# xmindflow/cenet

Hardware: AMD Instinct MI355X
Metric: training images/sec (224x224, 4-class) (higher is better)
Workload: dtype bf16

## Files before the change

cenet_amd/csrc/attn_diff.hip:

```cpp
#include "common.h"
#include "../../include/cenet_hip.h"
#include <cstdlib>

typedef bf16_t bf;
#define DA_NEG (-1.0e30f)
#define DA_LOG2E 1.4426950408889634f

#ifdef CENET_HOSTSIM_BUILD
__device__ __forceinline__ float da_exp2(float x) { return exp2f(x); }
__device__ __forceinline__ bool da_any(bool v) {
  int x = v ? 1 : 0;
#pragma unroll
  for (int o = 32; o > 0; o >>= 1) x |= __shfl_xor(x, o);
  return x != 0;
}
#else
__device__ __forceinline__ float da_exp2(float x) { return __builtin_amdgcn_exp2f(x); }
__device__ __forceinline__ bool da_any(bool v) { return __any(v); }
typedef short da_s4 __attribute__((ext_vector_type(4)));
#endif
__device__ __forceinline__ float da_max3(float a, float b, float c3) { return fmaxf(fmaxf(a, b), c3); }
__device__ __forceinline__ void da_wave_sync() {
#ifdef CENET_HOSTSIM_BUILD
  hipsim::wave_barrier();
#else
  __builtin_amdgcn_wave_barrier();
#endif
}

struct DiffArgs {
  const bf *q, *k, *v;
  bf* U;
  float* lse;
  const bf* dU;
  bf *dq, *dk, *dv;
  bf* aug;
  int B, H, N, hd;
  float scale;
  int bmul;
};

struct DaChunk {
  const bf* g;
  int lrow;
  int loff;
  unsigned fill;
};
__device__ __forceinline__ void da_fetch(const DaChunk& c, long tile_step, int rows_left, unsigned (&r)[4]) {
  r[0] = c.fill;
  r[1] = r[2] = r[3] = 0u;
  if (c.g && c.lrow < rows_left) memcpy(r, c.g + tile_step, 16);
  else if (!c.g) r[0] = 0u;
}
__device__ __forceinline__ bf16x8 da_rm(const bf* img, int pitch, int row, int col, int hh) {
  bf16x8 f;
  memcpy(&f, img + row * pitch + col + 8 * hh, 16);
  return f;
}
__device__ __forceinline__ bf16x8 da_tr(const bf* img, int pitch, int s2, int C0, int lane) {
  const int hh = lane >> 5;
  bf16x8 f;
#ifdef CENET_HOSTSIM_BUILD
  const int r = lane & 31;
#pragma unroll
  for (int j = 0; j < 8; ++j) f[j] = (short)img[(16 * s2 + 8 * (j >> 2) + 4 * hh + (j & 3)) * pitch + C0 + r];
#else
  const int g2 = (lane >> 4) & 1, i = lane & 15, q = i >> 2, p = i & 3;
  const bf* a0 = img + (16 * s2 + 4 * hh + q) * pitch + C0 + 16 * g2 + 4 * p;
  const da_s4 lo = __builtin_amdgcn_ds_read_tr16_b64_v4i16((da_s4 __attribute__((address_space(3)))*)a0);
  const da_s4 hi = __builtin_amdgcn_ds_read_tr16_b64_v4i16((da_s4 __attribute__((address_space(3)))*)(a0 + 8 * pitch));
  f[0] = lo[0], f[1] = lo[1], f[2] = lo[2], f[3] = lo[3];
  f[4] = hi[0], f[5] = hi[1], f[6] = hi[2], f[7] = hi[3];
#endif
  return f;
}
__device__ __forceinline__ bf16x8 da_ld8(const bf* p, bool ok) {
  bf16x8 f = {0, 0, 0, 0, 0, 0, 0, 0};
  if (ok) memcpy(&f, p, 16);
  return f;
}
__device__ __forceinline__ void da_half(unsigned (&r)[4], int s) {
  if (s) r[0] = r[2], r[1] = r[3];
  r[2] = r[3] = 0u;
}
__device__ __forceinline__ bf16x8 da_ld4h(const bf* pair, int s, bool ok) {
  unsigned u[4] = {0u, 0u, 0u, 0u};
  if (ok) {
    memcpy(u, pair, 16);
    da_half(u, s);
  }
  bf16x8 f;
  memcpy(&f, u, 16);
  return f;
}
__device__ __forceinline__ bf16x8 da_pack8(const f32x16& x, int s) {
  unsigned u[4];
#pragma unroll
  for (int j = 0; j < 4; ++j) u[j] = cenet_pack_bf2(x[8 * s + 2 * j], x[8 * s + 2 * j + 1]);
  bf16x8 f;
  memcpy(&f, u, 16);
  return f;
}
__device__ __forceinline__ int da_row(int reg, int hh) { return (reg & 3) + 8 * (reg >> 2) + 4 * hh; }
__device__ __forceinline__ f32x16 da_zero() {
  f32x16 z;
#pragma unroll
  for (int i = 0; i < 16; ++i) z[i] = 0.f;
  return z;
}
struct da_true { static constexpr bool value = true; };
struct da_false { static constexpr bool value = false; };
#define DA_MFMA(a, b, c) __builtin_amdgcn_mfma_f32_32x32x16_bf16((a), (b), (c), 0, 0, 0)

__device__ __forceinline__ void da_split3(float x, unsigned short* o) {
  const unsigned h = cenet_f2bf(x);
  const float r1 = x - cenet_bf2f(h);
  const unsigned m = cenet_f2bf(r1);
  const unsigned l = cenet_f2bf(r1 - cenet_bf2f(m));
  o[0] = (unsigned short)h, o[1] = (unsigned short)m, o[2] = (unsigned short)l;
}

template <int HDP>
struct DaGeo {
  static constexpr int DVP = 2 * HDP;
  static constexpr int KP = 2 * HDP + 8;
  static constexpr int VPT = DVP;
  static constexpr int VPR = DVP + 8;
  static constexpr int CK = 2 * HDP / 8, CV = DVP / 8;
};

template <int HDP, int QT, int MINB, bool ONE, bool H4 = false>
__global__ __launch_bounds__(256, MINB) void dattn_fwd_kernel(DiffArgs a) {
  typedef DaGeo<HDP> G;
  constexpr int NKS = HDP / 16, NDT = G::DVP / 32, NH = ONE ? 1 : 2;
  constexpr int KIMG = 32 * G::KP, VIMG = 32 * G::VPT + 64, IMG = KIMG + VIMG;
  constexpr int NCH = 32 * (G::CK + G::CV), CPT = (NCH + 255) / 256;
  __shared__ __attribute__((aligned(16))) bf lds[2 * IMG];
  const int tid = threadIdx.x, lane = tid & 63, wave = tid >> 6, r = lane & 31, hh = lane >> 5;
  const cenet_bid bid = cenet_xcd_block();
  const int b = bid.y / a.H, h = bid.y - b * a.H;
  const int q0 = (bid.x * 4 + wave) * (32 * QT);
  const int N = a.N, hd = a.hd, dv = 2 * hd, E = 2 * a.H * hd;
  const float c = a.scale * DA_LOG2E;
  const bf* qb = a.q + (long)b * a.bmul * N * E;
  const bf* kb = a.k + (long)b * a.bmul * N * E;
  const bf* vb = a.v + (long)b * a.bmul * N * (a.H * dv) + h * dv;

  DaChunk ch[CPT];
  int hs[CPT];
#pragma unroll
  for (int j = 0; j < CPT; ++j) {
    const int id = tid + 256 * j;
    ch[j].fill = 0u;
    hs[j] = -1;
    if (id >= NCH) {
      ch[j].g = nullptr;
      ch[j].lrow = 0;
      ch[j].loff = -1;
    } else if (id < 32 * G::CK) {
      const int row = id / G::CK, cc = id - row * G::CK, s = cc / (HDP / 8), c8 = cc - s * (HDP / 8);
      ch[j].lrow = row;
      ch[j].loff = row * G::KP + s * HDP + 8 * c8;
      ch[j].g = H4 ? (c8 == 0 ? kb + (long)row * E + 2 * h * hd : nullptr)
                   : (8 * c8 < hd ? kb + (long)row * E + (2 * h + s) * hd + 8 * c8 : nullptr);
      hs[j] = s;
    } else {
      const int id2 = id - 32 * G::CK, row = id2 / G::CV, c8 = id2 - row * G::CV;
      ch[j].lrow = row;
      ch[j].loff = KIMG + row * G::VPT + 8 * c8;
      ch[j].g = 8 * c8 < dv ? vb + (long)row * (a.H * dv) + 8 * c8 : nullptr;
    }
  }
  unsigned pre[CPT][4];
  auto fetch = [&](int k0) __attribute__((always_inline)) {
#pragma unroll
    for (int j = 0; j < CPT; ++j) {
      da_fetch(ch[j], (long)k0 * (ch[j].loff < KIMG ? E : a.H * dv), N - k0, pre[j]);
      if (H4 && hs[j] >= 0) da_half(pre[j], hs[j]);
    }
  };
  auto stage = [&](int buf) __attribute__((always_inline)) {
#pragma unroll
    for (int j = 0; j < CPT; ++j)
      if (ch[j].loff >= 0) memcpy(lds + buf * IMG + ch[j].loff, pre[j], 16);
  };

  bf16x8 qf[QT][2][NKS];
  f32x16 O[QT][NH][NDT];
  float m[QT][NH], l[QT][NH];
#pragma unroll
  for (int t = 0; t < QT; ++t) {
    const int qi = q0 + 32 * t + r < N ? q0 + 32 * t + r : N - 1;
#pragma unroll
    for (int s = 0; s < 2; ++s) {
#pragma unroll
      for (int ks = 0; ks < NKS; ++ks)
        qf[t][s][ks] = H4 ? da_ld4h(qb + (long)qi * E + 2 * h * hd, s, hh == 0)
                          : da_ld8(qb + (long)qi * E + (2 * h + s) * hd + 16 * ks + 8 * hh, 16 * ks + 8 * hh < hd);
    }
#pragma unroll
    for (int s = 0; s < NH; ++s) {
#pragma unroll
      for (int dt = 0; dt < NDT; ++dt) O[t][s][dt] = da_zero();
      m[t][s] = DA_NEG;
      l[t][s] = 0.f;
    }
  }
  fetch(0);
  stage(0);
  __syncthreads();
  int cur = 0;
  for (int k0 = 0; k0 < N; k0 += 32) {
    const bool more = k0 + 32 < N;
    if (more) fetch(k0 + 32);
    const bf* Kimg = lds + cur * IMG;
    const bf* Vimg = Kimg + KIMG;
    const int klim = N - k0;
    auto tile = [&](auto masked) __attribute__((always_inline)) {
      constexpr bool MASKED = decltype(masked)::value;
      constexpr bool LATE = HDP > 32;
      bf16x8 kf[LATE ? 1 : 2][NKS], vf[LATE ? 1 : NDT][2];
      if (!LATE) {
#pragma unroll
        for (int s = 0; s < 2; ++s)
#pragma unroll
          for (int ks = 0; ks < NKS; ++ks) kf[LATE ? 0 : s][ks] = da_rm(Kimg, G::KP, r, s * HDP + 16 * ks, hh);
#pragma unroll
        for (int dt = 0; dt < NDT; ++dt)
#pragma unroll
          for (int s2 = 0; s2 < 2; ++s2) vf[LATE ? 0 : dt][s2] = da_tr(Vimg, G::VPT, s2, 32 * dt, lane);
      }
#pragma unroll
      for (int t = 0; t < QT; ++t)
#pragma unroll
        for (int s = 0; s < NH; ++s) {
          f32x16 S = da_zero();
#pragma unroll
          for (int sp = (ONE ? 0 : s); sp <= (ONE ? 1 : s); ++sp)
#pragma unroll
            for (int ks = 0; ks < NKS; ++ks)
              S = DA_MFMA(LATE ? da_rm(Kimg, G::KP, r, sp * HDP + 16 * ks, hh) : kf[LATE ? 0 : sp][ks], qf[t][sp][ks], S);
          if (MASKED) {
#pragma unroll
            for (int i = 0; i < 16; ++i)
              if (da_row(i, hh) >= klim) S[i] = DA_NEG;
          }
          float mx = da_max3(S[0], S[1], S[2]);
#pragma unroll
          for (int i = 3; i < 15; i += 2) mx = da_max3(mx, S[i], S[i + 1]);
          mx = fmaxf(mx, S[15]);
          mx = fmaxf(mx, __shfl_xor(mx, 32));
          if (da_any(mx > m[t][s])) {
            const float mn = fmaxf(m[t][s], mx);
            const float alpha = da_exp2((m[t][s] - mn) * c);
            m[t][s] = mn;
            l[t][s] *= alpha;
#pragma unroll
            for (int dt = 0; dt < NDT; ++dt)
#pragma unroll
              for (int i = 0; i < 16; ++i) O[t][s][dt][i] *= alpha;
          }
          const float mc = m[t][s] * c;
          float rs = 0.f;
#pragma unroll
          for (int i = 0; i < 16; ++i) {
            const float p = da_exp2(S[i] * c - mc);
            S[i] = p;
            rs += p;
          }
          l[t][s] += rs;
          const bf16x8 p0 = da_pack8(S, 0), p1 = da_pack8(S, 1);
#pragma unroll
          for (int dt = 0; dt < NDT; ++dt) {
            O[t][s][dt] = DA_MFMA(LATE ? da_tr(Vimg, G::VPT, 0, 32 * dt, lane) : vf[LATE ? 0 : dt][0], p0, O[t][s][dt]);
            O[t][s][dt] = DA_MFMA(LATE ? da_tr(Vimg, G::VPT, 1, 32 * dt, lane) : vf[LATE ? 0 : dt][1], p1, O[t][s][dt]);
          }
        }
    };
    if (q0 < N) {
      if (klim < 32) tile(da_true());
      else tile(da_false());
    }
    if (more) stage(cur ^ 1);
    __syncthreads();
    cur ^= 1;
  }
  if (q0 >= N) return;
#pragma unroll
  for (int t = 0; t < QT; ++t) {
    const int qi = q0 + 32 * t + r;
#pragma unroll
    for (int s = 0; s < NH; ++s) {
      const float lt = l[t][s] + __shfl_xor(l[t][s], 32);
      const long hrow = ((long)b * NH * a.H + NH * h + s) * N + qi;
      if (qi < N) {
        const float inv = 1.f / lt;
        bf* up = a.U + hrow * dv;
#pragma unroll
        for (int dt = 0; dt < NDT; ++dt)
#pragma unroll
          for (int g = 0; g < 4; ++g) {
            const int f0 = 32 * dt + 8 * g + 4 * hh;
            if (f0 < dv) {
              float o[4];
#pragma unroll
              for (int i = 0; i < 4; ++i) o[i] = O[t][s][dt][4 * g + i] * inv;
              st4v(up + f0, o);
            }
          }
        if (hh == 0) a.lse[hrow] = m[t][s] * a.scale + logf(lt);
      }
    }
  }
}

template <int HDP, bool ONE, bool H4 = false>
__global__ __launch_bounds__(256, HDP > 32 ? 1 : (HDP <= 16 ? 3 : 2)) void dattn_bwd_dq_kernel(DiffArgs a) {
  typedef DaGeo<HDP> G;
  constexpr int NKS = HDP / 16, NKD = G::DVP / 16, NH = ONE ? 1 : 2;
  constexpr int NFT = (HDP + 31) / 32;
  constexpr int KIMG = 32 * G::KP + 64, VIMG = 32 * G::VPR, IMG = KIMG + VIMG;
  constexpr int NCH = 32 * (G::CK + G::CV), CPT = (NCH + 255) / 256;
  __shared__ __attribute__((aligned(16))) bf lds[2 * IMG];
  const int tid = threadIdx.x, lane = tid & 63, wave = tid >> 6, r = lane & 31, hh = lane >> 5;
  const cenet_bid bid = cenet_xcd_block();
  const int b = bid.y / a.H, h = bid.y - b * a.H;
  const int q0 = (bid.x * 4 + wave) * 32;
  const int N = a.N, hd = a.hd, dv = 2 * hd, E = 2 * a.H * hd;
  const float c = a.scale * DA_LOG2E;
  const bf* qb = a.q + (long)b * a.bmul * N * E;
  const bf* kb = a.k + (long)b * a.bmul * N * E;
  const bf* vb = a.v + (long)b * a.bmul * N * (a.H * dv) + h * dv;
  const int qi = q0 + r < N ? q0 + r : N - 1;

  DaChunk ch[CPT];
  int hs[CPT];
#pragma unroll
  for (int j = 0; j < CPT; ++j) {
    const int id = tid + 256 * j;
    ch[j].fill = 0u;
    hs[j] = -1;
    if (id >= NCH) {
      ch[j].g = nullptr;
      ch[j].lrow = 0;
      ch[j].loff = -1;
    } else if (id < 32 * G::CK) {
      const int row = id / G::CK, cc = id - row * G::CK, s = cc / (HDP / 8), c8 = cc - s * (HDP / 8);
      ch[j].lrow = row;
      ch[j].loff = row * G::KP + s * HDP + 8 * c8;
      ch[j].g = H4 ? (c8 == 0 ? kb + (long)row * E + 2 * h * hd : nullptr)
                   : (8 * c8 < hd ? kb + (long)row * E + (2 * h + s) * hd + 8 * c8 : nullptr);
      hs[j] = s;
    } else {
      const int id2 = id - 32 * G::CK, row = id2 / G::CV, c8 = id2 - row * G::CV;
      ch[j].lrow = row;
      ch[j].loff = KIMG + row * G::VPR + 8 * c8;
      ch[j].g = 8 * c8 < dv ? vb + (long)row * (a.H * dv) + 8 * c8 : nullptr;
    }
  }
  unsigned pre[CPT][4];
  auto fetch = [&](int k0) __attribute__((always_inline)) {
#pragma unroll
    for (int j = 0; j < CPT; ++j) {
      da_fetch(ch[j], (long)k0 * (ch[j].loff < KIMG ? E : a.H * dv), N - k0, pre[j]);
      if (H4 && hs[j] >= 0) da_half(pre[j], hs[j]);
    }
  };
  auto stage = [&](int buf) __attribute__((always_inline)) {
#pragma unroll
    for (int j = 0; j < CPT; ++j)
      if (ch[j].loff >= 0) memcpy(lds + buf * IMG + ch[j].loff, pre[j], 16);
  };

  bf16x8 qf[2][NKS], gf[NH][NKD];
  float lse2[NH], dl[NH];
  f32x16 dq[2][NFT];
#pragma unroll
  for (int s = 0; s < 2; ++s) {
#pragma unroll
    for (int ks = 0; ks < NKS; ++ks)
      qf[s][ks] = H4 ? da_ld4h(qb + (long)qi * E + 2 * h * hd, s, hh == 0)
                     : da_ld8(qb + (long)qi * E + (2 * h + s) * hd + 16 * ks + 8 * hh, 16 * ks + 8 * hh < hd);
#pragma unroll
    for (int ft = 0; ft < NFT; ++ft) dq[s][ft] = da_zero();
  }
#pragma unroll
  for (int s = 0; s < NH; ++s) {
    const long hrow = ((long)b * NH * a.H + NH * h + s) * N + qi;
    float acc = 0.f;
#pragma unroll
    for (int kd = 0; kd < NKD; ++kd) {
      const bool ok = 16 * kd + 8 * hh < dv;
      gf[s][kd] = da_ld8(a.dU + hrow * dv + 16 * kd + 8 * hh, ok);
      const bf16x8 uf = da_ld8(a.U + hrow * dv + 16 * kd + 8 * hh, ok);
#pragma unroll
      for (int j = 0; j < 8; ++j) acc += cenet_bf2f((unsigned short)gf[s][kd][j]) * cenet_bf2f((unsigned short)uf[j]);
    }
    acc += __shfl_xor(acc, 32);
    dl[s] = acc;
    const float lse = a.lse[hrow];
    lse2[s] = lse * DA_LOG2E;
    if (q0 + r < N) {
      unsigned short row8[8] = {0, 0, 0, 0, 0, 0, 0, 0};
      da_split3(hh == 0 ? lse / a.scale : acc, row8);
      memcpy(a.aug + hrow * 16 + 8 * hh, row8, 16);
    }
  }
  fetch(0);
  stage(0);
  __syncthreads();
  int cur = 0;
  for (int k0 = 0; k0 < N; k0 += 32) {
    const bool more = k0 + 32 < N;
    if (more) fetch(k0 + 32);
    const bf* Kimg = lds + cur * IMG;
    const bf* Vimg = Kimg + KIMG;
    const int klim = N - k0;
    auto tile = [&](auto masked) __attribute__((always_inline)) {
      constexpr bool MASKED = decltype(masked)::value;
      bf16x8 vf[NKD];
#pragma unroll
      for (int kd = 0; kd < NKD; ++kd) vf[kd] = da_rm(Vimg, G::VPR, r, 16 * kd, hh);
#pragma unroll
      for (int s = 0; s < NH; ++s) {
        constexpr bool INITD = HDP > 16;
        f32x16 S = da_zero(), dP;
#pragma unroll
        for (int i = 0; i < 16; ++i) dP[i] = INITD ? -dl[s] : 0.f;
#pragma unroll
        for (int sp = (ONE ? 0 : s); sp <= (ONE ? 1 : s); ++sp)
#pragma unroll
          for (int ks = 0; ks < NKS; ++ks) S = DA_MFMA(da_rm(Kimg, G::KP, r, sp * HDP + 16 * ks, hh), qf[sp][ks], S);
#pragma unroll
        for (int kd = 0; kd < NKD; ++kd) dP = DA_MFMA(vf[kd], gf[s][kd], dP);
#pragma unroll
        for (int i = 0; i < 16; ++i) {
          float p = da_exp2(S[i] * c - lse2[s]);
          if (MASKED && da_row(i, hh) >= klim) p = 0.f;
          S[i] = INITD ? p * dP[i] : p * (dP[i] - dl[s]);
        }
#pragma unroll
        for (int sp = (ONE ? 0 : s); sp <= (ONE ? 1 : s); ++sp)
#pragma unroll
          for (int s2 = 0; s2 < 2; ++s2) {
            const bf16x8 dsB = da_pack8(S, s2);
#pragma unroll
            for (int ft = 0; ft < NFT; ++ft)
              dq[sp][ft] = DA_MFMA(da_tr(Kimg, G::KP, s2, sp * HDP + 32 * ft, lane), dsB, dq[sp][ft]);
          }
      }
    };
    if (q0 < N) {
      if (klim < 32) tile(da_true());
      else tile(da_false());
    }
    if (more) stage(cur ^ 1);
    __syncthreads();
    cur ^= 1;
  }
  if (q0 + r < N) {
#pragma unroll
    for (int s = 0; s < 2; ++s) {
      bf* dp = a.dq + ((long)b * a.bmul * N + qi) * E + (2 * h + s) * hd;
#pragma unroll
      for (int ft = 0; ft < NFT; ++ft)
#pragma unroll
        for (int g = 0; g < (HDP < 32 ? HDP / 8 : 4); ++g) {
          const int d0 = 32 * ft + 8 * g + 4 * hh;
          if (d0 < hd) {
            float o[4];
#pragma unroll
            for (int i = 0; i < 4; ++i) o[i] = dq[s][ft][4 * g + i] * a.scale;
            st4v(dp + d0, o);
          }
        }
    }
  }
}

template <int HDP, bool ONE, bool H4 = false>
__global__ __launch_bounds__(256, HDP > 32 ? 1 : 2) void dattn_bwd_dkv_kernel(DiffArgs a) {
  typedef DaGeo<HDP> G;
  constexpr int NKS = HDP / 16, NKD = G::DVP / 16, NDT = G::DVP / 32, NH = ONE ? 1 : 2;
  constexpr int NFT = (HDP + 31) / 32;
  constexpr int AP = 40;
  constexpr int QIMG = 32 * G::KP + 64, GIMG = 32 * G::VPR + 64, AIMG = 32 * AP, IMG = QIMG + NH * GIMG + AIMG;
  constexpr int NCH = 32 * (G::CK + NH * G::CV + 2 * NH), CPT = (NCH + 255) / 256;
  __shared__ __attribute__((aligned(16))) bf lds[2 * IMG];
  const int tid = threadIdx.x, lane = tid & 63, wave = tid >> 6, r = lane & 31, hh = lane >> 5;
  const cenet_bid bid = cenet_xcd_block();
  const int b = bid.y / a.H, h = bid.y - b * a.H;
  const int k0 = (bid.x * 4 + wave) * 32;
  const int N = a.N, hd = a.hd, dv = 2 * hd, E = 2 * a.H * hd;
  const float c = a.scale * DA_LOG2E;
  const bf* qb = a.q + (long)b * a.bmul * N * E;
  const bf* kb = a.k + (long)b * a.bmul * N * E;
  const bf* vb = a.v + (long)b * a.bmul * N * (a.H * dv) + h * dv;
  const long hb0 = ((long)b * NH * a.H + NH * h) * N;
  const int ki = k0 + r < N ? k0 + r : N - 1;

  DaChunk ch[CPT];
  long gstep[CPT];
  int hs[CPT];
#pragma unroll
  for (int j = 0; j < CPT; ++j) {
    int id = tid + 256 * j;
    ch[j].fill = 0u;
    hs[j] = -1;
    gstep[j] = 0;
    if (id >= NCH) {
      ch[j].g = nullptr;
      ch[j].lrow = 0;
      ch[j].loff = -1;
    } else if (id < 32 * G::CK) {
      const int row = id / G::CK, cc = id - row * G::CK, s = cc / (HDP / 8), c8 = cc - s * (HDP / 8);
      ch[j].lrow = row;
      ch[j].loff = row * G::KP + s * HDP + 8 * c8;
      ch[j].g = H4 ? (c8 == 0 ? qb + (long)row * E + 2 * h * hd : nullptr)
                   : (8 * c8 < hd ? qb + (long)row * E + (2 * h + s) * hd + 8 * c8 : nullptr);
      hs[j] = s;
      gstep[j] = 32L * E;
    } else if ((id -= 32 * G::CK) < NH * 32 * G::CV) {
      const int s = id / (32 * G::CV), id2 = id - s * 32 * G::CV, row = id2 / G::CV, c8 = id2 - row * G::CV;
      ch[j].lrow = row;
      ch[j].loff = QIMG + s * GIMG + row * G::VPR + 8 * c8;
      ch[j].g = 8 * c8 < dv ? a.dU + (hb0 + (long)s * N + row) * dv + 8 * c8 : nullptr;
      gstep[j] = 32L * dv;
    } else {
      id -= NH * 32 * G::CV;
      const int row = id / (2 * NH), s = (id - row * 2 * NH) >> 1, kind = id & 1;
      ch[j].lrow = row;
      ch[j].loff = QIMG + NH * GIMG + row * AP + s * 16 + 8 * kind;
      ch[j].g = a.aug + (hb0 + (long)s * N + row) * 16 + 8 * kind;
      ch[j].fill = kind == 0 ? 0x7149u : 0u;
      gstep[j] = 32L * 16;
    }
  }
  unsigned pre[CPT][4];
  auto fetch = [&](int q0) __attribute__((always_inline)) {
#pragma unroll
    for (int j = 0; j < CPT; ++j) {
      da_fetch(ch[j], (q0 >> 5) * gstep[j], N - q0, pre[j]);
      if (H4 && hs[j] >= 0) da_half(pre[j], hs[j]);
    }
  };
  auto stage = [&](int buf) __attribute__((always_inline)) {
#pragma unroll
    for (int j = 0; j < CPT; ++j)
      if (ch[j].loff >= 0) memcpy(lds + buf * IMG + ch[j].loff, pre[j], 16);
  };

  bf16x8 kfB[2][NKS], vfB[NKD];
#pragma unroll
  for (int s = 0; s < 2; ++s)
#pragma unroll
    for (int ks = 0; ks < NKS; ++ks)
      kfB[s][ks] = H4 ? da_ld4h(kb + (long)ki * E + 2 * h * hd, s, hh == 0)
                      : da_ld8(kb + (long)ki * E + (2 * h + s) * hd + 16 * ks + 8 * hh, 16 * ks + 8 * hh < hd);
#pragma unroll
  for (int kd = 0; kd < NKD; ++kd) vfB[kd] = da_ld8(vb + (long)ki * (a.H * dv) + 16 * kd + 8 * hh, 16 * kd + 8 * hh < dv);
  bf16x8 negB = {0, 0, 0, 0, 0, 0, 0, 0};
  if (hh == 0) negB[0] = negB[1] = negB[2] = (short)0xBF80;
  f32x16 dK[2][NFT], dV[NDT];
#pragma unroll
  for (int s = 0; s < 2; ++s)
#pragma unroll
    for (int ft = 0; ft < NFT; ++ft) dK[s][ft] = da_zero();
#pragma unroll
  for (int dt = 0; dt < NDT; ++dt) dV[dt] = da_zero();

  fetch(0);
  stage(0);
  __syncthreads();
  int cur = 0;
  for (int q0 = 0; q0 < N; q0 += 32) {
    const bool more = q0 + 32 < N;
    if (more) fetch(q0 + 32);
    const bf* Qimg = lds + cur * IMG;
    const bf* Aimg = Qimg + QIMG + NH * GIMG;
    if (k0 < N) {
#pragma unroll
      for (int s = 0; s < NH; ++s) {
        const bf* Gimg = Qimg + QIMG + s * GIMG;
        f32x16 S = da_zero(), dP = da_zero();
#pragma unroll
        for (int sp = (ONE ? 0 : s); sp <= (ONE ? 1 : s); ++sp)
#pragma unroll
          for (int ks = 0; ks < NKS; ++ks) S = DA_MFMA(da_rm(Qimg, G::KP, r, sp * HDP + 16 * ks, hh), kfB[sp][ks], S);
#pragma unroll
        for (int kd = 0; kd < NKD; ++kd) dP = DA_MFMA(da_rm(Gimg, G::VPR, r, 16 * kd, hh), vfB[kd], dP);
        bf16x8 al = {0, 0, 0, 0, 0, 0, 0, 0}, ad = {0, 0, 0, 0, 0, 0, 0, 0};
        if (hh == 0) {
          memcpy(&al, Aimg + r * AP + s * 16, 16);
          memcpy(&ad, Aimg + r * AP + s * 16 + 8, 16);
        }
        S = DA_MFMA(al, negB, S);
        dP = DA_MFMA(ad, negB, dP);
#pragma unroll
        for (int i = 0; i < 16; ++i) {
          const float p = da_exp2(S[i] * c);
          S[i] = p;
          dP[i] = p * dP[i];
        }
#pragma unroll
        for (int s2 = 0; s2 < 2; ++s2) {
          const bf16x8 pB = da_pack8(S, s2), dsB = da_pack8(dP, s2);
#pragma unroll
          for (int dt = 0; dt < NDT; ++dt) dV[dt] = DA_MFMA(da_tr(Gimg, G::VPR, s2, 32 * dt, lane), pB, dV[dt]);
#pragma unroll
          for (int sp = (ONE ? 0 : s); sp <= (ONE ? 1 : s); ++sp)
#pragma unroll
            for (int ft = 0; ft < NFT; ++ft)
              dK[sp][ft] = DA_MFMA(da_tr(Qimg, G::KP, s2, sp * HDP + 32 * ft, lane), dsB, dK[sp][ft]);
        }
      }
    }
    if (more) stage(cur ^ 1);
    __syncthreads();
    cur ^= 1;
  }
  if (k0 + r < N) {
#pragma unroll
    for (int s = 0; s < 2; ++s) {
      bf* dp = a.dk + ((long)b * a.bmul * N + ki) * E + (2 * h + s) * hd;
#pragma unroll
      for (int ft = 0; ft < NFT; ++ft)
#pragma unroll
        for (int g = 0; g < (HDP < 32 ? HDP / 8 : 4); ++g) {
          const int d0 = 32 * ft + 8 * g + 4 * hh;
          if (d0 < hd) {
            float o[4];
#pragma unroll
            for (int i = 0; i < 4; ++i) o[i] = dK[s][ft][4 * g + i] * a.scale;
            st4v(dp + d0, o);
          }
        }
    }
    bf* dvp = a.dv + ((long)b * a.bmul * N + ki) * (a.H * dv) + h * dv;
#pragma unroll
    for (int dt = 0; dt < NDT; ++dt)
#pragma unroll
      for (int g = 0; g < 4; ++g) {
        const int f0 = 32 * dt + 8 * g + 4 * hh;
        if (f0 < dv) {
          float o[4];
#pragma unroll
          for (int i = 0; i < 4; ++i) o[i] = dV[dt][4 * g + i];
          st4v(dvp + f0, o);
        }
      }
  }
}

extern "C" int cenet_diffattn_heads_supported(int hd, int N) {
  return (hd == 4 || hd == 8 || hd == 16 || hd == 32 || hd == 40 || hd == 64) && N >= 1;
}
static bool da_hd40_p64() {
  const char* e = getenv("CENET_DATTN_HD40_HDP64");
  return e && e[0] == '1';
}
extern "C" long cenet_diffattn_heads_ws_bytes(int B, int H, int N) { return (long)B * 2 * H * N * 16 * 2; }

static int da_fill(DiffArgs& a, const cenet_diffattn_t* p) {
  if (!p || !p->q || !p->k || !p->v || !p->U || !p->lse) return CENET_EINVAL;
  if (p->B <= 0 || p->H <= 0 || p->N <= 0 || !cenet_diffattn_heads_supported(p->hd, p->N)) return CENET_EUNSUPPORTED;
  a.q = (const bf*)p->q; a.k = (const bf*)p->k; a.v = (const bf*)p->v;
  a.U = (bf*)p->U; a.lse = p->lse; a.dU = (const bf*)p->dU;
  a.dq = (bf*)p->dq; a.dk = (bf*)p->dk; a.dv = (bf*)p->dv; a.aug = (bf*)p->ws;
  a.B = p->B; a.H = p->H; a.N = p->N; a.hd = p->hd; a.scale = p->scale;
  a.bmul = p->batch_mul > 0 ? p->batch_mul : 1;
  const uintptr_t m = (uintptr_t)a.q | (uintptr_t)a.k | (uintptr_t)a.v | (uintptr_t)a.U | (uintptr_t)a.dU | (uintptr_t)a.dq |
                      (uintptr_t)a.dk | (uintptr_t)a.dv | (uintptr_t)a.aug;
  if (m & 15) return CENET_EINVAL;
  return CENET_OK;
}

extern "C" int cenet_diffattn_heads_fwd_bf16(const cenet_diffattn_t* p, hipStream_t stream) {
  DiffArgs a;
  const int rc = da_fill(a, p);
  if (rc != CENET_OK) return rc;
  const int bh = a.B * a.H;
  if (a.hd == 4) {
    CENET_LAUNCH((dattn_fwd_kernel<16, 1, 3, false, true>), dim3(cdiv(a.N, 128), bh), dim3(256), stream, a);
  } else if (a.hd <= 16) {
    static const int v = getenv("CENET_DATTN_QT2") ? 2 : 1;
    if (v == 2 && a.N >= 1024) CENET_LAUNCH((dattn_fwd_kernel<16, 2, 2, false>), dim3(cdiv(a.N, 256), bh), dim3(256), stream, a);
    else CENET_LAUNCH((dattn_fwd_kernel<16, 1, 3, false>), dim3(cdiv(a.N, 128), bh), dim3(256), stream, a);
  } else if (a.hd <= 32) {
    CENET_LAUNCH((dattn_fwd_kernel<32, 1, 2, false>), dim3(cdiv(a.N, 128), bh), dim3(256), stream, a);
  } else if (a.hd == 40 && !da_hd40_p64()) {
    CENET_LAUNCH((dattn_fwd_kernel<48, 1, 1, false>), dim3(cdiv(a.N, 128), bh), dim3(256), stream, a);
  } else {
    CENET_LAUNCH((dattn_fwd_kernel<64, 1, 1, false>), dim3(cdiv(a.N, 128), bh), dim3(256), stream, a);
  }
  CENET_CHECK_LAUNCH();
  return CENET_OK;
}

extern "C" int cenet_diffattn_heads_bwd_bf16(const cenet_diffattn_t* p, hipStream_t stream) {
  DiffArgs a;
  const int rc = da_fill(a, p);
  if (rc != CENET_OK) return rc;
  if (!a.dU || !a.dq || !a.dk || !a.dv || !a.aug) return CENET_EINVAL;
  const dim3 grid(cdiv(a.N, 128), a.B * a.H);
  if (a.hd == 4) {
    CENET_LAUNCH((dattn_bwd_dq_kernel<16, false, true>), grid, dim3(256), stream, a);
    CENET_LAUNCH((dattn_bwd_dkv_kernel<16, false, true>), grid, dim3(256), stream, a);
  } else if (a.hd <= 16) {
    CENET_LAUNCH((dattn_bwd_dq_kernel<16, false>), grid, dim3(256), stream, a);
    CENET_LAUNCH((dattn_bwd_dkv_kernel<16, false>), grid, dim3(256), stream, a);
  } else if (a.hd <= 32) {
    CENET_LAUNCH((dattn_bwd_dq_kernel<32, false>), grid, dim3(256), stream, a);
    CENET_LAUNCH((dattn_bwd_dkv_kernel<32, false>), grid, dim3(256), stream, a);
  } else if (a.hd == 40 && !da_hd40_p64()) {
    CENET_LAUNCH((dattn_bwd_dq_kernel<48, false>), grid, dim3(256), stream, a);
    CENET_LAUNCH((dattn_bwd_dkv_kernel<48, false>), grid, dim3(256), stream, a);
  } else {
    CENET_LAUNCH((dattn_bwd_dq_kernel<64, false>), grid, dim3(256), stream, a);
    CENET_LAUNCH((dattn_bwd_dkv_kernel<64, false>), grid, dim3(256), stream, a);
  }
  CENET_CHECK_LAUNCH();
  return CENET_OK;
}

extern "C" long cenet_attn64_ws_bytes(int B, int H, int N) { return (long)B * H * N * 16 * 2; }

static int da_fill64(DiffArgs& a, const cenet_diffattn_t* p) {
  if (!p || !p->q || !p->k || !p->v || !p->U || !p->lse) return CENET_EINVAL;
  if (p->B <= 0 || p->H <= 0 || p->N <= 0 || (p->hd != 64 && p->hd != 128)) return CENET_EUNSUPPORTED;
  a.q = (const bf*)p->q; a.k = (const bf*)p->k; a.v = (const bf*)p->v;
  a.U = (bf*)p->U; a.lse = p->lse; a.dU = (const bf*)p->dU;
  a.dq = (bf*)p->dq; a.dk = (bf*)p->dk; a.dv = (bf*)p->dv; a.aug = (bf*)p->ws;
  a.B = p->B; a.H = p->H; a.N = p->N; a.hd = p->hd / 2; a.scale = p->scale;
  a.bmul = p->batch_mul > 0 ? p->batch_mul : 1;
  const uintptr_t m = (uintptr_t)a.q | (uintptr_t)a.k | (uintptr_t)a.v | (uintptr_t)a.U | (uintptr_t)a.dU | (uintptr_t)a.dq |
                      (uintptr_t)a.dk | (uintptr_t)a.dv | (uintptr_t)a.aug;
  if (m & 15) return CENET_EINVAL;
  return CENET_OK;
}

extern "C" int cenet_attn64_fwd_bf16(const cenet_diffattn_t* p, hipStream_t stream) {
  DiffArgs a;
  const int rc = da_fill64(a, p);
  if (rc != CENET_OK) return rc;
  if (a.hd == 32) CENET_LAUNCH((dattn_fwd_kernel<32, 1, 2, true>), dim3(cdiv(a.N, 128), a.B * a.H), dim3(256), stream, a);
  else CENET_LAUNCH((dattn_fwd_kernel<64, 1, 1, true>), dim3(cdiv(a.N, 128), a.B * a.H), dim3(256), stream, a);
  CENET_CHECK_LAUNCH();
  return CENET_OK;
}

extern "C" int cenet_attn64_bwd_bf16(const cenet_diffattn_t* p, hipStream_t stream) {
  DiffArgs a;
  const int rc = da_fill64(a, p);
  if (rc != CENET_OK) return rc;
  if (!a.dU || !a.dq || !a.dk || !a.dv || !a.aug) return CENET_EINVAL;
  const dim3 grid(cdiv(a.N, 128), a.B * a.H);
  if (a.hd == 32) {
    CENET_LAUNCH((dattn_bwd_dq_kernel<32, true>), grid, dim3(256), stream, a);
    CENET_LAUNCH((dattn_bwd_dkv_kernel<32, true>), grid, dim3(256), stream, a);
  } else {
    CENET_LAUNCH((dattn_bwd_dq_kernel<64, true>), grid, dim3(256), stream, a);
    CENET_LAUNCH((dattn_bwd_dkv_kernel<64, true>), grid, dim3(256), stream, a);
  }
  CENET_CHECK_LAUNCH();
  return CENET_OK;
}

struct SraArgs {
  const bf *q, *kv, *o, *dout;
  const float* lse;
  bf* dq;
  float* dkv;
  bf* dkv_bf;
  int B, H, Nq, Nk, C, tiles;
  float scale;
};

template <int NKB, bool DQ, bool DKV>
__global__ __launch_bounds__(256, DKV ? 1 : 2) void sra_bwd_kernel(SraArgs a) {
  constexpr int KP = 72, AP = 40;
  constexpr int KVIMG = NKB * 64 * KP, QIMG = 32 * KP + 64, AIMG = 32 * AP;
  constexpr int WIMG = 2 * QIMG + AIMG;
  constexpr int LDS_EL = (DQ ? 2 * KVIMG : 0) + (DKV ? 4 * WIMG : 0);
  static_assert(!DKV || LDS_EL * 2 >= 64 * 128 * 4, "the dK/dV reduction block reuses the images");
  static_assert(NKB == 1 || !DKV, "dK / dV accumulators exist for one 64-key block");
  __shared__ __attribute__((aligned(16))) bf lds[LDS_EL];
  const int tid = threadIdx.x, lane = tid & 63, wave = tid >> 6, r = lane & 31, hh = lane >> 5;
  const cenet_bid bid = cenet_xcd_block();
  const int b = bid.y / a.H, h = bid.y - b * a.H;
  const int key0 = DQ ? 0 : 64 * bid.z;
  const int C = a.C, Nq = a.Nq;
  const int Nk = DQ ? a.Nk : (a.Nk - key0 < 64 ? a.Nk - key0 : 64);
  const float c = a.scale * DA_LOG2E;
  const bf* qb = a.q + (long)b * Nq * C + h * 64;
  const bf* ob = a.o + (long)b * Nq * C + h * 64;
  const bf* gb = a.dout + (long)b * Nq * C + h * 64;
  const bf* kb = a.kv + ((long)b * a.Nk + key0) * 2 * C + h * 64;
  const bf* vb = kb + C;
  bf* Kimg = lds;
  bf* Vimg = lds + KVIMG;
  bf* Qimg = lds + (DQ ? 2 * KVIMG : 0) + wave * WIMG;
  bf* Gimg = Qimg + QIMG;
  bf* Aimg = Gimg + QIMG;
  if (DQ) {
    for (int id = tid; id < 2 * NKB * 64 * 8; id += 256) {
      const int which = id / (NKB * 512), rem = id - which * (NKB * 512), row = rem >> 3, c8 = rem & 7;
      unsigned v4[4] = {0u, 0u, 0u, 0u};
      if (row < Nk) memcpy(v4, (which ? vb : kb) + (long)row * 2 * C + 8 * c8, 16);
      memcpy((which ? Vimg : Kimg) + row * KP + 8 * c8, v4, 16);
    }
  }
  bf16x8 kfB[2][4], vfB[2][4];
  if (DKV) {
#pragma unroll
    for (int kt = 0; kt < 2; ++kt)
#pragma unroll
      for (int ks = 0; ks < 4; ++ks) {
        const int key = 32 * kt + r;
        kfB[kt][ks] = da_ld8(kb + (long)(key < Nk ? key : 0) * 2 * C + 16 * ks + 8 * hh, key < Nk);
        vfB[kt][ks] = da_ld8(vb + (long)(key < Nk ? key : 0) * 2 * C + 16 * ks + 8 * hh, key < Nk);
      }
  }
  bf16x8 negB = {0, 0, 0, 0, 0, 0, 0, 0};
  if (hh == 0) negB[0] = negB[1] = negB[2] = (short)0xBF80;
  f32x16 dK[2][2], dV[2][2];
#pragma unroll
  for (int kt = 0; kt < 2; ++kt)
#pragma unroll
    for (int dt = 0; dt < 2; ++dt) dK[kt][dt] = dV[kt][dt] = da_zero();
  __syncthreads();

  const int q00 = (bid.x * 4 + wave) * 32 * a.tiles;
  for (int t = 0; t < a.tiles; ++t) {
    const int q0 = q00 + 32 * t;
    if (q0 >= Nq) break;
    const int qi = q0 + r < Nq ? q0 + r : Nq - 1;
    const bool qok = q0 + r < Nq;
    bf16x8 qf[4], gf[4];
    float acc = 0.f;
#pragma unroll
    for (int ks = 0; ks < 4; ++ks) {
      qf[ks] = da_ld8(qb + (long)qi * C + 16 * ks + 8 * hh, true);
      gf[ks] = da_ld8(gb + (long)qi * C + 16 * ks + 8 * hh, true);
      const bf16x8 uf = da_ld8(ob + (long)qi * C + 16 * ks + 8 * hh, true);
#pragma unroll
      for (int j = 0; j < 8; ++j) acc += cenet_bf2f((unsigned short)gf[ks][j]) * cenet_bf2f((unsigned short)uf[j]);
      if (DKV) {
        bf16x8 qz = qf[ks], gz = gf[ks];
        if (!qok) qz = gz = bf16x8{0, 0, 0, 0, 0, 0, 0, 0};
        memcpy(Qimg + r * KP + 16 * ks + 8 * hh, &qz, 16);
        memcpy(Gimg + r * KP + 16 * ks + 8 * hh, &gz, 16);
      }
    }
    acc += __shfl_xor(acc, 32);
    const float delta = acc;
    const float lse = a.lse[((long)b * a.H + h) * Nq + qi];
    const float lse2 = lse * DA_LOG2E;
    if (DKV) {
      unsigned short row8[8] = {0, 0, 0, 0, 0, 0, 0, 0};
      da_split3(hh == 0 ? (qok ? lse / a.scale : 1.0e30f) : (qok ? delta : 0.f), row8);
      memcpy(Aimg + r * AP + 8 * hh, row8, 16);
    }
    f32x16 dq[2] = {da_zero(), da_zero()};
#pragma unroll
    for (int kt = 0; kt < (DQ ? 2 * NKB : 0); ++kt) {
      if (32 * kt >= Nk) continue;
      const bf* Kt = Kimg + 32 * kt * KP;
      const bf* Vt = Vimg + 32 * kt * KP;
      f32x16 S = da_zero(), dP = da_zero();
#pragma unroll
      for (int ks = 0; ks < 4; ++ks) {
        S = DA_MFMA(da_rm(Kt, KP, r, 16 * ks, hh), qf[ks], S);
        dP = DA_MFMA(da_rm(Vt, KP, r, 16 * ks, hh), gf[ks], dP);
      }
#pragma unroll
      for (int i = 0; i < 16; ++i) {
        float pv = da_exp2(S[i] * c - lse2);
        if (32 * kt + da_row(i, hh) >= Nk) pv = 0.f;
        S[i] = pv * (dP[i] - delta);
      }
#pragma unroll
      for (int dt = 0; dt < 2; ++dt)
#pragma unroll
        for (int s2 = 0; s2 < 2; ++s2) dq[dt] = DA_MFMA(da_tr(Kt, KP, s2, 32 * dt, lane), da_pack8(S, s2), dq[dt]);
    }
    if (DQ && qok) {
      bf* dp = a.dq + ((long)b * Nq + qi) * C + h * 64;
#pragma unroll
      for (int dt = 0; dt < 2; ++dt)
#pragma unroll
        for (int g = 0; g < 4; ++g) {
          float o4[4];
#pragma unroll
          for (int i = 0; i < 4; ++i) o4[i] = dq[dt][4 * g + i] * a.scale;
          st4v(dp + 32 * dt + 8 * g + 4 * hh, o4);
        }
    }
    if (!DKV) continue;
    da_wave_sync();
    bf16x8 al = {0, 0, 0, 0, 0, 0, 0, 0}, ad = {0, 0, 0, 0, 0, 0, 0, 0};
    if (hh == 0) {
      memcpy(&al, Aimg + r * AP, 16);
      memcpy(&ad, Aimg + r * AP + 8, 16);
    }
#pragma unroll
    for (int kt = 0; kt < 2; ++kt) {
      if (32 * kt >= Nk) continue;
      f32x16 S = da_zero(), dP = da_zero();
#pragma unroll
      for (int ks = 0; ks < 4; ++ks) {
        S = DA_MFMA(da_rm(Qimg, KP, r, 16 * ks, hh), kfB[kt][ks], S);
        dP = DA_MFMA(da_rm(Gimg, KP, r, 16 * ks, hh), vfB[kt][ks], dP);
      }
      S = DA_MFMA(al, negB, S);
      dP = DA_MFMA(ad, negB, dP);
      const bool kok = 32 * kt + r < Nk;
#pragma unroll
      for (int i = 0; i < 16; ++i) {
        const float pv = kok ? da_exp2(S[i] * c) : 0.f;
        S[i] = pv;
        dP[i] = pv * dP[i];
      }
#pragma unroll
      for (int s2 = 0; s2 < 2; ++s2) {
        const bf16x8 pB = da_pack8(S, s2), dsB = da_pack8(dP, s2);
#pragma unroll
        for (int dt = 0; dt < 2; ++dt) {
          dV[kt][dt] = DA_MFMA(da_tr(Gimg, KP, s2, 32 * dt, lane), pB, dV[kt][dt]);
          dK[kt][dt] = DA_MFMA(da_tr(Qimg, KP, s2, 32 * dt, lane), dsB, dK[kt][dt]);
        }
      }
    }
  }
  if (!DKV) return;
  float* red = (float*)lds;
  __syncthreads();
  for (int w = 0; w < 4; ++w) {
    if (wave == w) {
#pragma unroll
      for (int kt = 0; kt < 2; ++kt)
#pragma unroll
        for (int dt = 0; dt < 2; ++dt)
#pragma unroll
          for (int i = 0; i < 16; ++i) {
            const int key = 32 * kt + r, f = 32 * dt + da_row(i, hh);
            if (w == 0) {
              red[f * 64 + key] = dK[kt][dt][i];
              red[(64 + f) * 64 + key] = dV[kt][dt][i];
            } else {
              red[f * 64 + key] += dK[kt][dt][i];
              red[(64 + f) * 64 + key] += dV[kt][dt][i];
            }
          }
    }
    __syncthreads();
  }
  if (a.dkv_bf) {
    bf* dkvb = a.dkv_bf + ((long)b * a.Nk + key0) * 2 * C + h * 64;
    for (int i = tid; i < Nk * 128; i += 256) {
      const int key = i >> 7, f = i & 127;
      const float v = red[f * 64 + key];
      if (f < 64) stf(dkvb + (long)key * 2 * C + f, v * a.scale);
      else stf(dkvb + (long)key * 2 * C + C + (f - 64), v);
    }
    return;
  }
  float* dkv = a.dkv + ((long)b * a.Nk + key0) * 2 * C + h * 64;
  for (int i = tid; i < Nk * 128; i += 256) {
    const int key = i >> 7, f = i & 127;
    const float v = red[f * 64 + key];
    if (f < 64) atomicAdd(&dkv[(long)key * 2 * C + f], v * a.scale);
    else atomicAdd(&dkv[(long)key * 2 * C + C + (f - 64)], v);
  }
}

struct SraFwdArgs {
  const bf *q, *kv;
  bf* o;
  float* lse;
  int B, H, Nq, Nk, C, tiles;
  float scale;
};

__global__ __launch_bounds__(256, 2) void sra_fwd_kernel(SraFwdArgs a) {
  constexpr int KP = 72, KVIMG = 64 * KP;
  __shared__ __attribute__((aligned(16))) bf lds[2 * KVIMG + 64];
  const int tid = threadIdx.x, lane = tid & 63, wave = tid >> 6, r = lane & 31, hh = lane >> 5;
  const cenet_bid bid = cenet_xcd_block();
  const int b = bid.y / a.H, h = bid.y - b * a.H;
  const int C = a.C, Nq = a.Nq, Nk = a.Nk;
  const float c = a.scale * DA_LOG2E;
  const bf* qb = a.q + (long)b * Nq * C + h * 64;
  bf* ob = a.o + (long)b * Nq * C + h * 64;
  const bf* kb = a.kv + (long)b * Nk * 2 * C + h * 64;
  const bf* vb = kb + C;
  bf* Kimg = lds;
  bf* Vimg = lds + KVIMG;
  for (int id = tid; id < 2 * 64 * 8; id += 256) {
    const int which = id >> 9, rem = id & 511, row = rem >> 3, c8 = rem & 7;
    unsigned v4[4] = {0u, 0u, 0u, 0u};
    if (row < Nk) memcpy(v4, (which ? vb : kb) + (long)row * 2 * C + 8 * c8, 16);
    memcpy((which ? Vimg : Kimg) + row * KP + 8 * c8, v4, 16);
  }
  __syncthreads();
  const int q00 = (bid.x * 4 + wave) * 32 * a.tiles;
  for (int t = 0; t < a.tiles; ++t) {
    const int q0 = q00 + 32 * t;
    if (q0 >= Nq) break;
    const int qi = q0 + r < Nq ? q0 + r : Nq - 1;
    bf16x8 qf[4];
#pragma unroll
    for (int ks = 0; ks < 4; ++ks) qf[ks] = da_ld8(qb + (long)qi * C + 16 * ks + 8 * hh, true);
    f32x16 S[2];
#pragma unroll
    for (int kt = 0; kt < 2; ++kt) {
      S[kt] = da_zero();
      if (32 * kt < Nk) {
#pragma unroll
        for (int ks = 0; ks < 4; ++ks) S[kt] = DA_MFMA(da_rm(Kimg + 32 * kt * KP, KP, r, 16 * ks, hh), qf[ks], S[kt]);
      }
#pragma unroll
      for (int i = 0; i < 16; ++i)
        if (32 * kt + da_row(i, hh) >= Nk) S[kt][i] = DA_NEG;
    }
    float mx = DA_NEG;
#pragma unroll
    for (int kt = 0; kt < 2; ++kt)
#pragma unroll
      for (int i = 0; i < 16; ++i) mx = fmaxf(mx, S[kt][i]);
    mx = fmaxf(mx, __shfl_xor(mx, 32));
    const float mc = mx * c;
    float l = 0.f;
#pragma unroll
    for (int kt = 0; kt < 2; ++kt)
#pragma unroll
      for (int i = 0; i < 16; ++i) {
        const float pv = da_exp2(S[kt][i] * c - mc);
        S[kt][i] = pv;
        l += pv;
      }
    l += __shfl_xor(l, 32);
    f32x16 O[2] = {da_zero(), da_zero()};
#pragma unroll
    for (int kt = 0; kt < 2; ++kt) {
      if (32 * kt >= Nk) continue;
      const bf* Vt = Vimg + 32 * kt * KP;
#pragma unroll
      for (int s2 = 0; s2 < 2; ++s2) {
        const bf16x8 pB = da_pack8(S[kt], s2);
#pragma unroll
        for (int dt = 0; dt < 2; ++dt) O[dt] = DA_MFMA(da_tr(Vt, KP, s2, 32 * dt, lane), pB, O[dt]);
      }
    }
    if (q0 + r < Nq) {
      const float inv = 1.f / l;
      bf* op = ob + (long)qi * C;
#pragma unroll
      for (int dt = 0; dt < 2; ++dt)
#pragma unroll
        for (int g = 0; g < 4; ++g) {
          float o4[4];
#pragma unroll
          for (int i = 0; i < 4; ++i) o4[i] = O[dt][4 * g + i] * inv;
          st4v(op + 32 * dt + 8 * g + 4 * hh, o4);
        }
      if (hh == 0) a.lse[((long)b * a.H + h) * Nq + qi] = mx * a.scale + logf(l);
    }
  }
}

extern "C" int cenet_sra_attn_fwd_bf16(const bf* q, const bf* kv, bf* o, float* lse, int B, int H, int Nq, int Nk, float scale,
                                       hipStream_t stream) {
  if (!q || !kv || !o || !lse || B <= 0 || H <= 0 || Nq <= 0) return CENET_EINVAL;
  if (!(Nk >= 1 && Nk <= 64)) return CENET_EUNSUPPORTED;
  if ((((uintptr_t)q | (uintptr_t)kv | (uintptr_t)o) & 15) != 0) return CENET_EINVAL;
  SraFwdArgs a;
  a.q = q; a.kv = kv; a.o = o; a.lse = lse; a.B = B; a.H = H; a.Nq = Nq; a.Nk = Nk; a.C = 64 * H; a.scale = scale;
  static const char* e = getenv("CENET_SRA_FWD_TILES");
  int tiles = 1;
  while (tiles < 8 && (long)cdiv(Nq, 128 * tiles) * B * H > 1024) ++tiles;
  if (e) tiles = atoi(e);
  a.tiles = tiles < 1 ? 1 : tiles;
  CENET_LAUNCH(sra_fwd_kernel, dim3(cdiv(Nq, 128 * a.tiles), B * H), dim3(256), stream, a);
  CENET_CHECK_LAUNCH();
  return CENET_OK;
}

extern "C" int cenet_sra_attn_bwd_supported(int hd, int Nk) { return hd == 64 && Nk >= 1 && Nk <= 64; }
extern "C" int cenet_sra_attn_bwd_blocks_supported(int hd, int Nk) { return hd == 64 && Nk > 64 && Nk <= 256; }

static int sra_tiles(int B, int H, int Nq) {
  static const char* e = getenv("CENET_SRA_TILES");
  int tiles = 1;
  while (tiles < 8 && (long)cdiv(Nq, 128 * tiles) * B * H > 256) ++tiles;
  if (e) tiles = atoi(e);
  return tiles < 1 ? 1 : tiles;
}
extern "C" int cenet_sra_attn_bwd_direct_supported(int B, int H, int Nq, int Nk) {
  return cenet_sra_attn_bwd_supported(64, Nk) && B > 0 && H > 0 && Nq > 0 && cdiv(Nq, 128 * sra_tiles(B, H, Nq)) == 1;
}

static int sra_bwd_launch(const bf* q, const bf* kv, const bf* o, const bf* dout, const float* lse, bf* dq, float* dkv, bf* dkv_bf,
                          int B, int H, int Nq, int Nk, float scale, hipStream_t stream) {
  if (!q || !kv || !o || !dout || !lse || !dq || (!dkv && !dkv_bf) || B <= 0 || H <= 0 || Nq <= 0) return CENET_EINVAL;
  const bool blocks = cenet_sra_attn_bwd_blocks_supported(64, Nk);
  if (!cenet_sra_attn_bwd_supported(64, Nk) && !blocks) return CENET_EUNSUPPORTED;
  if ((((uintptr_t)q | (uintptr_t)kv | (uintptr_t)o | (uintptr_t)dout | (uintptr_t)dq) & 15) != 0) return CENET_EINVAL;
  SraArgs a;
  a.q = q; a.kv = kv; a.o = o; a.dout = dout; a.lse = lse; a.dq = dq; a.dkv = dkv; a.dkv_bf = dkv_bf;
  a.B = B; a.H = H; a.Nq = Nq; a.Nk = Nk; a.C = 64 * H; a.scale = scale;
  a.tiles = sra_tiles(B, H, Nq);
  if (blocks) {
    if (dkv_bf) return CENET_EUNSUPPORTED;
    int tq = 1;
    while (tq < 8 && (long)cdiv(Nq, 128 * tq) * B * H > 512) ++tq;
    a.tiles = tq;
    CENET_LAUNCH((sra_bwd_kernel<4, true, false>), dim3(cdiv(Nq, 128 * tq), B * H), dim3(256), stream, a);
    const int nkb = cdiv(Nk, 64);
    int tk = 1;
    while (tk < 16 && (long)cdiv(Nq, 128 * tk) * B * H * nkb > 256) ++tk;
    a.tiles = tk;
    CENET_LAUNCH((sra_bwd_kernel<1, false, true>), dim3(cdiv(Nq, 128 * tk), B * H, nkb), dim3(256), stream, a);
    CENET_CHECK_LAUNCH();
    return CENET_OK;
  }
  if (dkv_bf && cdiv(Nq, 128 * a.tiles) != 1) return CENET_EUNSUPPORTED;
  CENET_LAUNCH((sra_bwd_kernel<1, true, true>), dim3(cdiv(Nq, 128 * a.tiles), B * H), dim3(256), stream, a);
  CENET_CHECK_LAUNCH();
  return CENET_OK;
}

extern "C" int cenet_sra_attn_bwd_bf16(const bf* q, const bf* kv, const bf* o, const bf* dout, const float* lse, bf* dq, float* dkv,
                                       int B, int H, int Nq, int Nk, float scale, hipStream_t stream) {
  if (!dkv) return CENET_EINVAL;
  return sra_bwd_launch(q, kv, o, dout, lse, dq, dkv, nullptr, B, H, Nq, Nk, scale, stream);
}

extern "C" int cenet_sra_attn_bwd_direct_bf16(const bf* q, const bf* kv, const bf* o, const bf* dout, const float* lse, bf* dq,
                                              bf* dkv, int B, int H, int Nq, int Nk, float scale, hipStream_t stream) {
  if (!dkv) return CENET_EINVAL;
  return sra_bwd_launch(q, kv, o, dout, lse, dq, nullptr, dkv, B, H, Nq, Nk, scale, stream);
}
```

Baseline: 1828.

## Add lean register-light fused SRA backward path with prefetch and split reduction

For the fused dQ+dK/dV SRA backward instance, a lean variant reads K/V from the LDS images instead of holding them in registers. It recomputes the dQ path from the LDS Q/G images and prefetches the next tile's q/dout/o/lse during the dK/dV phase. This lets it run with two blocks per CU instead of one. The final dK/dV reduction is split across two LDS buffers in two turns, and the bf16 output store is vectorised. The tile heuristic also changes to favour larger tiles, and the env lookup is no longer cached. The cost is redundant LDS reads and extra wave syncs.

Result: no change. 1838 (median of 6 runs) (+0.6%).

```diff
diff --git a/cenet_amd/csrc/attn_diff.hip b/cenet_amd/csrc/attn_diff.hip
--- a/cenet_amd/csrc/attn_diff.hip
+++ b/cenet_amd/csrc/attn_diff.hip
@@ -777,13 +777,15 @@
 };
 
 template <int NKB, bool DQ, bool DKV>
-__global__ __launch_bounds__(256, DKV ? 1 : 2) void sra_bwd_kernel(SraArgs a) {
+__global__ __launch_bounds__(256, (DKV && !DQ) ? 1 : 2) void sra_bwd_kernel(SraArgs a) {
+  constexpr bool LEAN = DQ && DKV;
   constexpr int KP = 72, AP = 40;
   constexpr int KVIMG = NKB * 64 * KP, QIMG = 32 * KP + 64, AIMG = 32 * AP;
   constexpr int WIMG = 2 * QIMG + AIMG;
   constexpr int LDS_EL = (DQ ? 2 * KVIMG : 0) + (DKV ? 4 * WIMG : 0);
   static_assert(!DKV || LDS_EL * 2 >= 64 * 128 * 4, "the dK/dV reduction block reuses the images");
   static_assert(NKB == 1 || !DKV, "dK / dV accumulators exist for one 64-key block");
+  static_assert(!LEAN || LDS_EL * 2 >= 2 * 64 * 128 * 4, "the lean instance reduces through two blocks");
   __shared__ __attribute__((aligned(16))) bf lds[LDS_EL];
   const int tid = threadIdx.x, lane = tid & 63, wave = tid >> 6, r = lane & 31, hh = lane >> 5;
   const cenet_bid bid = cenet_xcd_block();
@@ -802,6 +804,20 @@
   bf* Qimg = lds + (DQ ? 2 * KVIMG : 0) + wave * WIMG;
   bf* Gimg = Qimg + QIMG;
   bf* Aimg = Gimg + QIMG;
+  const int q00 = (bid.x * 4 + wave) * 32 * a.tiles;
+  const long lrow0 = ((long)b * a.H + h) * Nq;
+  bf16x8 qn[4], gn[4], un[4];
+  float lsen = 0.f;
+  if (LEAN && q00 < Nq) {
+    const int qi = q00 + r < Nq ? q00 + r : Nq - 1;
+#pragma unroll
+    for (int ks = 0; ks < 4; ++ks) {
+      qn[ks] = da_ld8(qb + (long)qi * C + 16 * ks + 8 * hh, true);
+      gn[ks] = da_ld8(gb + (long)qi * C + 16 * ks + 8 * hh, true);
+      un[ks] = da_ld8(ob + (long)qi * C + 16 * ks + 8 * hh, true);
+    }
+    lsen = a.lse[lrow0 + qi];
+  }
   if (DQ) {
     for (int id = tid; id < 2 * NKB * 64 * 8; id += 256) {
       const int which = id / (NKB * 512), rem = id - which * (NKB * 512), row = rem >> 3, c8 = rem & 7;
@@ -811,7 +827,7 @@
     }
   }
   bf16x8 kfB[2][4], vfB[2][4];
-  if (DKV) {
+  if (DKV && !LEAN) {
 #pragma unroll
     for (int kt = 0; kt < 2; ++kt)
 #pragma unroll
@@ -830,19 +846,19 @@
     for (int dt = 0; dt < 2; ++dt) dK[kt][dt] = dV[kt][dt] = da_zero();
   __syncthreads();
 
-  const int q00 = (bid.x * 4 + wave) * 32 * a.tiles;
   for (int t = 0; t < a.tiles; ++t) {
     const int q0 = q00 + 32 * t;
     if (q0 >= Nq) break;
     const int qi = q0 + r < Nq ? q0 + r : Nq - 1;
     const bool qok = q0 + r < Nq;
+    if (LEAN) da_wave_sync();
     bf16x8 qf[4], gf[4];
     float acc = 0.f;
 #pragma unroll
     for (int ks = 0; ks < 4; ++ks) {
-      qf[ks] = da_ld8(qb + (long)qi * C + 16 * ks + 8 * hh, true);
-      gf[ks] = da_ld8(gb + (long)qi * C + 16 * ks + 8 * hh, true);
-      const bf16x8 uf = da_ld8(ob + (long)qi * C + 16 * ks + 8 * hh, true);
+      qf[ks] = LEAN ? qn[ks] : da_ld8(qb + (long)qi * C + 16 * ks + 8 * hh, true);
+      gf[ks] = LEAN ? gn[ks] : da_ld8(gb + (long)qi * C + 16 * ks + 8 * hh, true);
+      const bf16x8 uf = LEAN ? un[ks] : da_ld8(ob + (long)qi * C + 16 * ks + 8 * hh, true);
 #pragma unroll
       for (int j = 0; j < 8; ++j) acc += cenet_bf2f((unsigned short)gf[ks][j]) * cenet_bf2f((unsigned short)uf[j]);
       if (DKV) {
@@ -854,16 +870,17 @@
     }
     acc += __shfl_xor(acc, 32);
     const float delta = acc;
-    const float lse = a.lse[((long)b * a.H + h) * Nq + qi];
+    const float lse = LEAN ? lsen : a.lse[lrow0 + qi];
     const float lse2 = lse * DA_LOG2E;
     if (DKV) {
       unsigned short row8[8] = {0, 0, 0, 0, 0, 0, 0, 0};
       da_split3(hh == 0 ? (qok ? lse / a.scale : 1.0e30f) : (qok ? delta : 0.f), row8);
       memcpy(Aimg + r * AP + 8 * hh, row8, 16);
     }
+    if (LEAN) da_wave_sync();
     f32x16 dq[2] = {da_zero(), da_zero()};
 #pragma unroll
-    for (int kt = 0; kt < (DQ ? 2 * NKB : 0); ++kt) {
+    for (int kt = 0; kt < (DQ && !LEAN ? 2 * NKB : 0); ++kt) {
       if (32 * kt >= Nk) continue;
       const bf* Kt = Kimg + 32 * kt * KP;
       const bf* Vt = Vimg + 32 * kt * KP;
@@ -884,7 +901,51 @@
 #pragma unroll
         for (int s2 = 0; s2 < 2; ++s2) dq[dt] = DA_MFMA(da_tr(Kt, KP, s2, 32 * dt, lane), da_pack8(S, s2), dq[dt]);
     }
-    if (DQ && qok) {
+    if (LEAN) {
+      bf16x8 dsB[2][2];
+#pragma unroll
+      for (int kt = 0; kt < 2; ++kt) {
+        dsB[kt][0] = dsB[kt][1] = bf16x8{0, 0, 0, 0, 0, 0, 0, 0};
+        if (32 * kt >= Nk) continue;
+        const bf* Kt = Kimg + 32 * kt * KP;
+        const bf* Vt = Vimg + 32 * kt * KP;
+        f32x16 S = da_zero(), dP = da_zero();
+#pragma unroll
+        for (int ks = 0; ks < 4; ++ks) {
+          S = DA_MFMA(da_rm(Kt, KP, r, 16 * ks, hh), da_rm(Qimg, KP, r, 16 * ks, hh), S);
+          dP = DA_MFMA(da_rm(Vt, KP, r, 16 * ks, hh), da_rm(Gimg, KP, r, 16 * ks, hh), dP);
+        }
+#pragma unroll
+        for (int i = 0; i < 16; ++i) {
+          float pv = da_exp2(S[i] * c - lse2);
+          if (32 * kt + da_row(i, hh) >= Nk) pv = 0.f;
+          S[i] = pv * (dP[i] - delta);
+        }
+        dsB[kt][0] = da_pack8(S, 0);
+        dsB[kt][1] = da_pack8(S, 1);
+      }
+      bf* dp = a.dq + ((long)b * Nq + qi) * C + h * 64;
+#pragma unroll
+      for (int dt = 0; dt < 2; ++dt) {
+        f32x16 dqh = da_zero();
+#pragma unroll
+        for (int kt = 0; kt < 2; ++kt) {
+          if (32 * kt >= Nk) continue;
+#pragma unroll
+          for (int s2 = 0; s2 < 2; ++s2) dqh = DA_MFMA(da_tr(Kimg + 32 * kt * KP, KP, s2, 32 * dt, lane), dsB[kt][s2], dqh);
+        }
+        if (qok) {
+#pragma unroll
+          for (int g = 0; g < 4; ++g) {
+            float o4[4];
+#pragma unroll
+            for (int i = 0; i < 4; ++i) o4[i] = dqh[4 * g + i] * a.scale;
+            st4v(dp + 32 * dt + 8 * g + 4 * hh, o4);
+          }
+        }
+      }
+    }
+    if (DQ && !LEAN && qok) {
       bf* dp = a.dq + ((long)b * Nq + qi) * C + h * 64;
 #pragma unroll
       for (int dt = 0; dt < 2; ++dt)
@@ -897,9 +958,20 @@
         }
     }
     if (!DKV) continue;
-    da_wave_sync();
+    if (LEAN && t + 1 < a.tiles && q0 + 32 < Nq) {
+      const int qa = q0 + 32 + r < Nq ? q0 + 32 + r : Nq - 1;
+      const long off = (long)qa * C + 8 * hh;
+#pragma unroll
+      for (int ks = 0; ks < 4; ++ks) {
+        qn[ks] = da_ld8(qb + (off + 16 * ks), true);
+        gn[ks] = da_ld8(gb + (off + 16 * ks), true);
+        un[ks] = da_ld8(ob + (off + 16 * ks), true);
+      }
+      lsen = a.lse[lrow0 + qa];
+    }
+    if (!LEAN) da_wave_sync();
     bf16x8 al = {0, 0, 0, 0, 0, 0, 0, 0}, ad = {0, 0, 0, 0, 0, 0, 0, 0};
-    if (hh == 0) {
+    if (!LEAN && hh == 0) {
       memcpy(&al, Aimg + r * AP, 16);
       memcpy(&ad, Aimg + r * AP + 8, 16);
     }
@@ -909,11 +981,23 @@
       f32x16 S = da_zero(), dP = da_zero();
 #pragma unroll
       for (int ks = 0; ks < 4; ++ks) {
-        S = DA_MFMA(da_rm(Qimg, KP, r, 16 * ks, hh), kfB[kt][ks], S);
-        dP = DA_MFMA(da_rm(Gimg, KP, r, 16 * ks, hh), vfB[kt][ks], dP);
-      }
-      S = DA_MFMA(al, negB, S);
-      dP = DA_MFMA(ad, negB, dP);
+        S = DA_MFMA(da_rm(Qimg, KP, r, 16 * ks, hh), LEAN ? da_rm(Kimg + 32 * kt * KP, KP, r, 16 * ks, hh) : kfB[kt][ks], S);
+        dP = DA_MFMA(da_rm(Gimg, KP, r, 16 * ks, hh), LEAN ? da_rm(Vimg + 32 * kt * KP, KP, r, 16 * ks, hh) : vfB[kt][ks], dP);
+      }
+      if (LEAN && hh == 0) {
+        memcpy(&al, Aimg + r * AP, 16);
+        memcpy(&ad, Aimg + r * AP + 8, 16);
+      }
+      bf16x8 nB = negB;
+      if (LEAN) {
+        int m1 = hh == 0 ? 0xBF80 : 0;
+#ifndef CENET_HOSTSIM_BUILD
+        asm volatile("" : "+v"(m1));
+#endif
+        nB = bf16x8{(short)m1, (short)m1, (short)m1, 0, 0, 0, 0, 0};
+      }
+      S = DA_MFMA(al, nB, S);
+      dP = DA_MFMA(ad, nB, dP);
       const bool kok = 32 * kt + r < Nk;
 #pragma unroll
       for (int i = 0; i < 16; ++i) {
@@ -933,10 +1017,12 @@
     }
   }
   if (!DKV) return;
-  float* red = (float*)lds;
+  constexpr int TURNS = LEAN ? 2 : 4;
+  float* red = (float*)lds + (LEAN ? (wave & 1) * 64 * 128 : 0);
+  const bool idle = LEAN && q00 >= Nq;
   __syncthreads();
-  for (int w = 0; w < 4; ++w) {
-    if (wave == w) {
+  for (int w = 0; w < TURNS; ++w) {
+    if ((LEAN ? wave >> 1 : wave) == w && !(idle && w > 0)) {
 #pragma unroll
       for (int kt = 0; kt < 2; ++kt)
 #pragma unroll
@@ -955,13 +1041,21 @@
     }
     __syncthreads();
   }
+  red = (float*)lds;
+  if (LEAN) {
+    for (int i = tid; i < 64 * 128; i += 256) red[i] += red[64 * 128 + i];
+    __syncthreads();
+  }
   if (a.dkv_bf) {
     bf* dkvb = a.dkv_bf + ((long)b * a.Nk + key0) * 2 * C + h * 64;
-    for (int i = tid; i < Nk * 128; i += 256) {
-      const int key = i >> 7, f = i & 127;
-      const float v = red[f * 64 + key];
-      if (f < 64) stf(dkvb + (long)key * 2 * C + f, v * a.scale);
-      else stf(dkvb + (long)key * 2 * C + C + (f - 64), v);
+    for (int i = tid; i < Nk * 32; i += 256) {
+      const int key = i >> 5, f = 4 * (i & 31);
+      float v4[4] = {red[f * 64 + key], red[(f + 1) * 64 + key], red[(f + 2) * 64 + key], red[(f + 3) * 64 + key]};
+      if (f < 64) {
+#pragma unroll
+        for (int j = 0; j < 4; ++j) v4[j] *= a.scale;
+      }
+      st4v(dkvb + (long)key * 2 * C + (f < 64 ? f : C + f - 64), v4);
     }
     return;
   }
@@ -1090,9 +1184,10 @@
 extern "C" int cenet_sra_attn_bwd_blocks_supported(int hd, int Nk) { return hd == 64 && Nk > 64 && Nk <= 256; }
 
 static int sra_tiles(int B, int H, int Nq) {
-  static const char* e = getenv("CENET_SRA_TILES");
+  const char* e = getenv("CENET_SRA_TILES");
   int tiles = 1;
-  while (tiles < 8 && (long)cdiv(Nq, 128 * tiles) * B * H > 256) ++tiles;
+  while (tiles < 8 && (long)cdiv(Nq, 128 * tiles) * B * H > 512) ++tiles;
+  if (cdiv(Nq, 128 * tiles) == 2 && (long)B * H >= 128) tiles *= 2;
   if (e) tiles = atoi(e);
   return tiles < 1 ? 1 : tiles;
 }
@@ -1125,6 +1220,7 @@
     return CENET_OK;
   }
   if (dkv_bf && cdiv(Nq, 128 * a.tiles) != 1) return CENET_EUNSUPPORTED;
+  if (dkv_bf && ((uintptr_t)dkv_bf & 15) != 0) return CENET_EINVAL;
   CENET_LAUNCH((sra_bwd_kernel<1, true, true>), dim3(cdiv(Nq, 128 * a.tiles), B * H), dim3(256), stream, a);
   CENET_CHECK_LAUNCH();
   return CENET_OK;
```
